# nv-tlabs/LION

Measured on NVIDIA H100. Metric: shapes/sec (1000-step DDPM, 2048 latent pts, B=32), higher is better.
Workload: dtype tf32 (fp32 storage/accumulate)

## Files before the change

### include/lion_b200.h

```cpp
#ifndef LION_B200_H
#define LION_B200_H
#include <stddef.h>
#ifdef __cplusplus
extern "C" {
#endif

typedef struct LionCtx LionCtx;
typedef struct LionModel LionModel;

int lion_version(void);
const char* lion_last_error(void);
int lion_ctx_create(int device, LionCtx** out);
int lion_ctx_destroy(LionCtx* ctx);
int lion_ctx_last_launches(LionCtx* ctx);
unsigned lion_ctx_generation(LionCtx* ctx);
int lion_ctx_timeline(LionCtx* ctx, unsigned long long* t_ns, char* names, int max_entries);
size_t lion_ctx_arena_bytes(LionCtx* ctx);
size_t lion_workspace_bytes(LionCtx* ctx);

int lion_avg_voxelize(const float* features, const int* coords, float* out, int* ind, int* cnt,
                      int B, int C, int N, int r, void* stream);
int lion_trilinear_devoxelize(const float* grid, const float* coords, float* out, int* inds, float* wgts,
                              int B, int C, int N, int r, int is_training, void* stream);
int lion_furthest_point_sampling(const float* coords, int* idx, int B, int N, int M, void* stream);
int lion_gather(const float* features, const int* idx, float* out, int B, int C, int N, int M, void* stream);
int lion_ball_query(const float* centers, const float* points, int* out, int B, int N, int M, float radius, int K,
                    void* stream);
int lion_grouping(const float* features, const int* idx, float* out, int B, int C, int N, int M, int U, void* stream);
int lion_three_nn_interpolate(const float* points, const float* centers, const float* centers_features, float* out,
                              int* idx, float* wgt, int B, int C, int N, int M, void* stream);
int lion_voxel_coords(const float* coords, float* norm_coords, int* vox, int B, int N, int r, int normalize, float eps,
                      void* stream);

int lion_avg_voxelize_backward(const float* grad_y , const int* ind , const int* cnt ,
                               float* grad_x , int B, int C, int N, int r, void* stream);
int lion_trilinear_devoxelize_backward(const float* grad_y , const int* inds , const float* wgts ,
                                       float* grad_x , int B, int C, int N, int r, void* stream);
int lion_grouping_backward(const float* grad_y , const int* idx , float* grad_x , int B, int C,
                           int N, int M, int U, void* stream);
int lion_three_nn_interpolate_backward(const float* grad_y , const int* idx , const float* wgt ,
                                       float* grad_x , int B, int C, int N, int M, void* stream);
int lion_gather_backward(const float* grad_y , const int* idx , float* grad_x , int B, int C, int N,
                         int M, void* stream);

enum { LION_KIND_UNET = 1, LION_KIND_PVCONV = 2, LION_KIND_SA = 3, LION_KIND_FP = 4, LION_KIND_ATTN = 5,
       LION_KIND_SHARED_MLP = 6, LION_KIND_GLOBAL_PRIOR = 7, LION_KIND_ADAGN = 8, LION_KIND_CONV3D = 9,
       LION_KIND_STYLE_ENC = 10 };
// ... 70 lines not shown
```

### lion_b200/_lib.py

```python
import ctypes as C
import os
import threading

import torch

_HERE = os.path.dirname(os.path.abspath(__file__))
LIB_PATH = os.path.join(_HERE, "csrc", "liblion_b200.so")


class LionError(RuntimeError):
    pass


_lib = None
_lock = threading.Lock()
c_f = C.c_void_p


def _proto(lib):
    i, f, sz, vp = C.c_int, C.c_float, C.c_size_t, C.c_void_p
    P = lambda *a: list(a)
    sig = {
        "lion_version": ([], i),
        "lion_last_error": ([], C.c_char_p),
        "lion_ctx_create": (P(i, C.POINTER(vp)), i),
        "lion_ctx_destroy": (P(vp), i),
        "lion_ctx_last_launches": (P(vp), i),
        "lion_ctx_arena_bytes": (P(vp), sz),
        "lion_ctx_generation": (P(vp), C.c_uint),
        "lion_ctx_timeline": (P(vp, vp, vp, i), i),
        "lion_avg_voxelize": (P(vp, vp, vp, vp, vp, i, i, i, i, vp), i),
        "lion_trilinear_devoxelize": (P(vp, vp, vp, vp, vp, i, i, i, i, i, vp), i),
        "lion_furthest_point_sampling": (P(vp, vp, i, i, i, vp), i),
        "lion_gather": (P(vp, vp, vp, i, i, i, i, vp), i),
        "lion_ball_query": (P(vp, vp, vp, i, i, i, f, i, vp), i),
        "lion_grouping": (P(vp, vp, vp, i, i, i, i, i, vp), i),
        "lion_three_nn_interpolate": (P(vp, vp, vp, vp, vp, vp, i, i, i, i, vp), i),
        "lion_voxel_coords": (P(vp, vp, vp, i, i, i, i, f, vp), i),
        "lion_avg_voxelize_backward": (P(vp, vp, vp, vp, i, i, i, i, vp), i),
        "lion_trilinear_devoxelize_backward": (P(vp, vp, vp, vp, i, i, i, i, vp), i),
        "lion_grouping_backward": (P(vp, vp, vp, i, i, i, i, i, vp), i),
        "lion_three_nn_interpolate_backward": (P(vp, vp, vp, vp, i, i, i, i, vp), i),
        "lion_gather_backward": (P(vp, vp, vp, i, i, i, i, vp), i),
        "lion_model_create": (P(vp, i, C.POINTER(i), i, C.POINTER(vp), i, C.POINTER(vp)), i),
        "lion_model_destroy": (P(vp), i),
        "lion_model_refresh": (P(vp), i),
        "lion_unet_forward": (P(vp, vp, vp, vp, vp, vp, i, i, vp), i),
        "lion_unet_cache_style": (P(vp, vp, vp, i, vp), i),
        "lion_style_encoder_forward": (P(vp, vp, vp, i, i, vp), i),
        "lion_pvconv_fwd": (P(vp, vp, vp, vp, vp, i, i, vp), i),
        "lion_sa_module_fwd": (P(vp, vp, vp, vp, vp, vp, i, i, vp), i),
        "lion_fp_module_fwd": (P(vp, vp, vp, vp, vp, vp, vp, i, i, i, vp), i),
        "lion_linear_attention_fwd": (P(vp, vp, vp, i, i, vp), i),
        "lion_shared_mlp_fwd": (P(vp, vp, vp, vp, i, i, vp), i),
        "lion_global_prior_forward": (P(vp, vp, vp, vp, vp, i, vp), i),
        "lion_adagn_fwd": (P(vp, vp, vp, vp, i, i, vp), i),
        "lion_se3d_fwd": (P(vp, vp, vp, vp, vp, i, i, i, vp), i),
        "lion_swish_fwd": (P(vp, vp, sz, vp), i),
        "lion_ddpm_update": (P(vp, vp, vp, vp, vp, vp, f, sz, vp, i, vp), i),
        "lion_ddpm_set_step": (P(vp, vp, i, i, vp), i),
# ... 178 lines not shown
```

### lion_b200/csrc/common.cuh

```cuda
#pragma once
#include <cuda_runtime.h>
#include <cstdint>
#include <cstdio>
#include <cstdarg>
#include <cstring>
#include <string>
#include <vector>
#include <mutex>

namespace lion {

enum : int { LION_OK = 0, LION_ERR_CUDA = -1, LION_ERR_ARG = -2, LION_ERR_OOM = -3, LION_ERR_STATE = -4 };

void set_error(const char* fmt, ...);
const char* get_error();

#define LION_CHECK_CUDA(expr)                                                          \
  do {                                                                                 \
    cudaError_t _e = (expr);                                                           \
    if (_e != cudaSuccess) {                                                           \
      lion::set_error("%s:%d: %s -> %s", __FILE__, __LINE__, #expr, cudaGetErrorString(_e)); \
      return lion::LION_ERR_CUDA;                                                      \
    }                                                                                  \
  } while (0)

#define LION_REQUIRE(cond, ...)                                                        \
  do {                                                                                 \
    if (!(cond)) {                                                                     \
      lion::set_error(__VA_ARGS__);                                                    \
      return lion::LION_ERR_ARG;                                                       \
    }                                                                                  \
  } while (0)

#define LION_TRY(expr)                                                                 \
  do {                                                                                 \
    int _r = (expr);                                                                   \
    if (_r != 0) return _r;                                                            \
  } while (0)

constexpr int LION_MAX_STAMPS = 256;
struct Ctx {
  int device = 0;
  int num_sms = 132;
  int l2_bytes = 50 << 20;
  cudaStream_t stream = nullptr;
  cudaStream_t aux = nullptr;
  char* base = nullptr;
  char* zgrid = nullptr;
  size_t zgrid_cap = 0, zgrid_need = 0;
  size_t cap = 0;
  size_t off = 0;
  size_t peak = 0;
  unsigned generation = 0;
  std::mutex* mu = nullptr;
  bool dry = false;
  int launches = 0;
  int conv_smem_cap = 0;
  unsigned long long* d_stamps = nullptr;
  int n_stamps = 0;
  char stamp_names[LION_MAX_STAMPS][24];

  void reset() { off = 0; peak = 0; launches = 0; zgrid_need = 0; n_stamps = 0; }
  void* alloc(size_t bytes) {
    size_t a = (off + 255) & ~size_t(255);
    off = a + bytes;
    if (off > peak) peak = off;
    if (dry) return (void*)(uintptr_t)(0x1000 + a);
    return base + a;
  }
  template <typename T> T* alloc_n(size_t n) { return (T*)alloc(n * sizeof(T)); }
  size_t mark() const { return off; }
  void release(size_t m) { off = m; }
};

int ctx_reserve(Ctx* c, size_t bytes);

#define LION_LAUNCH_ON(ctx, stream, kernel, grid, block, smem, ...)                    \
  do {                                                                                 \
    if (!(ctx)->dry) {                                                                 \
      kernel<<<(grid), (block), (smem), (stream)>>>(__VA_ARGS__);                      \
      (ctx)->launches++;                                                               \
    }                                                                                  \
  } while (0)
#define LION_LAUNCH(ctx, kernel, grid, block, smem, ...) LION_LAUNCH_ON(ctx, (ctx)->stream, kernel, grid, block, smem, __VA_ARGS__)

static __global__ void k_stamp(unsigned long long* p) {
  unsigned long long t;
  asm volatile("mov.u64 %0, %%globaltimer;" : "=l"(t));
  *p = t;
}
// ... 82 lines not shown
```

### lion_b200/csrc/conv_tc.cu

```cuda
#include <algorithm>

#include "common.cuh"
#include "model.cuh"
#include "wgmma.cuh"

namespace lion {
namespace tc {

using namespace sm90;

constexpr int CONSUMER_WARPS = 8;
constexpr int THREADS = 32 * CONSUMER_WARPS + 32;
constexpr int MAX_A_STAGES = 16;
constexpr int MAX_B_STAGES = 4;
constexpr int OCC_SMEM = 1024;
__host__ __device__ constexpr int tiles_per_item(int NT) { return NT <= 32 ? 4 : (NT <= 64 ? 2 : 1); }
constexpr int SMEM_BIAS = 128 * 4, SMEM_BARS = 64 * 8 + 128;
__host__ __device__ constexpr int smem_stat(int NT) { return CONSUMER_WARPS * 2 * NT * 4; }
__host__ __device__ constexpr int smem_pool(int NT, int TPG) { return TPG == 1 ? CONSUMER_WARPS * 2 * NT * 4 : 0; }
__host__ __device__ constexpr int smem_fixed(int NT, int TPG) {
  return SMEM_BIAS + smem_stat(NT) + smem_pool(NT, TPG) + SMEM_BARS + OCC_SMEM;
}

struct Params {
  const float4* in; const float* w; const float* bias; float4* out; double* ssum; double* ssq;
  int Gin, Gout_store, cout_pad;
  int rows;
  int p_begin, p_end;
  int ntile;
  int ntg, tpg;
  int tg_off[3];
  int tap_off[9];
  int r, rp, nzb, npl, nblk, ib;
  int halo;
  int KG, nchunk;
  int NT;
  int G;
  int B;
  int a_stage_bytes, b_stage_bytes, stage_rows;
  int a_stages;
  int b_stages;
  const unsigned char* occ;
  int occ_stride;
  float* pool_mm;
  int sched;
};

__host__ __device__ __forceinline__ int block_row(int k, int rp, int nzb, int npl) {
  const int x = k / npl, rem = k - x * npl, yb = rem / nzb, zb = rem - yb * nzb;
  return ((x + 1) * rp + 1 + 8 * yb) * rp + 1 + 8 * zb;
}

template <int KG, int TPG, int NT>
__device__ __forceinline__ void issue_stage(float* d, uint32_t a_addr, uint32_t b_addr, uint32_t a_pitch, uint32_t a_sbo,
                                            const int* tap_off) {
  const uint64_t a0 = make_desc(a_addr, a_pitch, a_sbo), b0 = make_desc(b_addr, NT * 16, 128);
#pragma unroll
  for (int t = 0; t < TPG; ++t) {
    const uint64_t at = a0 + (uint64_t)(int64_t)(TPG == 1 ? 0 : tap_off[t]);
#pragma unroll
    for (int ks = 0; ks < KG / 2; ++ks)
      wgmma_tf32<NT>(d, at + (uint64_t)((ks * 2 * a_pitch) >> 4), b0 + (uint64_t)(((t * KG + ks * 2) * NT * 16) >> 4), 1);
  }
}


struct Items {
  long long u, u_end; int ntile_total, B, G;
  int mode, m, q, n_p, n_q, c_i, i, big, k;
  __device__ __forceinline__ bool next(int& nt, long long& v0, int& ntile) {
    const long long per_nt = (long long)B * ntile_total;
    if (mode) {
      while (u >= u_end) {
        if (k >= m) return false;
        const int a0 = q * k / m, a1 = q * (k + 1) / m, b0 = (q + 1) * k / m, b1 = (q + 1) * (k + 1) / m;
        u = (long long)n_q * a0 + (long long)n_p * b0 + (long long)(i - c_i) * (a1 - a0) + (long long)c_i * (b1 - b0);
        u_end = u + (big ? b1 - b0 : a1 - a0);
        ++k;
      }
      nt = (int)(u / per_nt);
      v0 = u - (long long)nt * per_nt;
      const long long lim = (long long)(nt + 1) * per_nt;
      const long long e = u_end < lim ? u_end : lim;
      ntile = (int)(e - u);
      u = e;
      return true;
    }
    if (u >= u_end) return false;
    nt = (int)(u / per_nt);
    v0 = u - (long long)nt * per_nt;
    long long run = per_nt - v0;
    if (u_end - u < run) run = u_end - u;
    const long long k2 = (run + G - 1) / G;
    ntile = (int)((run + k2 - 1) / k2);
    u += ntile;
// ... 15 lines not shown
}

__device__ __forceinline__ void halo_mask(int p_lo, int rp, bool& ok_lo, bool& ok_hi) {
  const int p_hi = p_lo + 8;
  const int z0 = p_lo % rp, y0 = (p_lo / rp) % rp, z1 = p_hi % rp, y1 = (p_hi / rp) % rp;
  ok_lo = ok_lo && z0 >= 1 && z0 <= rp - 2 && y0 >= 1 && y0 <= rp - 2;
  ok_hi = ok_hi && z1 >= 1 && z1 <= rp - 2 && y1 >= 1 && y1 <= rp - 2;
}
template <int NT>
__device__ __forceinline__ void stat_add(float* s_stat, int cw, int lane, int col, float x0, float x1, float x2, float x3) {
  const float s0 = red8<0>(x0 + x2), s1 = red8<0>(x1 + x3);
  const float q0 = red8<0>(fmaf(x0, x0, x2 * x2)), q1 = red8<0>(fmaf(x1, x1, x3 * x3));
  if (lane < 4) {
    float* st = s_stat + (cw * 2) * NT + col;
    st[0] += s0; st[1] += s1; st[NT] += q0; st[NT + 1] += q1;
  }
}
template <int NT>
__device__ __forceinline__ void stat_flush(const Params& P, float* s_stat, int et, int b, int n0) {
  asm volatile("bar.sync 1, 256;" ::: "memory");
  if (et < NT) {
    float s = 0.f, qq = 0.f;
#pragma unroll
    for (int w = 0; w < CONSUMER_WARPS; ++w) {
      s += s_stat[(w * 2 + 0) * NT + et]; qq += s_stat[(w * 2 + 1) * NT + et];
      s_stat[(w * 2 + 0) * NT + et] = 0.0f; s_stat[(w * 2 + 1) * NT + et] = 0.0f;
    }
    atomicAdd(P.ssum + (size_t)b * P.cout_pad + n0 + et, (double)s);
    atomicAdd(P.ssq + (size_t)b * P.cout_pad + n0 + et, (double)qq);
  }
  asm volatile("bar.sync 1, 256;" ::: "memory");
}

template <int KG, int TPG, int NT, bool BLK>
__global__ void __launch_bounds__(THREADS, 1) k_conv_tc(Params P) {
  constexpr int GT = tiles_per_item(NT);
  constexpr int NACC = NT / 2;
  extern __shared__ __align__(128) uint8_t smem[];
  uint8_t* sA = smem;
  const int A_STAGES = P.a_stages;
  uint8_t* sB = sA + (size_t)A_STAGES * P.a_stage_bytes;
  const int B_STAGES = P.b_stages;
  float* s_bias = (float*)(sB + (size_t)B_STAGES * P.b_stage_bytes);
  float* s_stat = s_bias + 128;
  float* s_pool = s_stat + CONSUMER_WARPS * 2 * NT;
  uint64_t* bars = (uint64_t*)((uint8_t*)s_stat + smem_stat(NT) + smem_pool(NT, TPG));
  volatile uint32_t* s_skip = (volatile uint32_t*)(bars + 64);
  uint8_t* s_occ = (uint8_t*)(bars + 64) + 128;
  const int tid = threadIdx.x, warp = tid >> 5, lane = tid & 31;

  const uint32_t bar_full_a = smem_u32(bars), bar_empty_a = smem_u32(bars + MAX_A_STAGES);
  const uint32_t bar_full_b = smem_u32(bars + 2 * MAX_A_STAGES), bar_empty_b = smem_u32(bars + 2 * MAX_A_STAGES + MAX_B_STAGES);

  if (P.Gin % KG != 0)
    for (int i = tid; i < A_STAGES * P.a_stage_bytes / 16; i += THREADS) ((float4*)sA)[i] = make_float4(0.f, 0.f, 0.f, 0.f);
  for (int i = tid; i < CONSUMER_WARPS * 2 * NT; i += THREADS) s_stat[i] = 0.0f;
  if (tid == 0) {
    for (int i = 0; i < A_STAGES; ++i) { mbar_init(bar_full_a + 8 * i, 1); mbar_init(bar_empty_a + 8 * i, CONSUMER_WARPS); }
    for (int i = 0; i < B_STAGES; ++i) { mbar_init(bar_full_b + 8 * i, 1); mbar_init(bar_empty_b + 8 * i, CONSUMER_WARPS); }
    asm volatile("fence.mbarrier_init.release.cluster;" ::: "memory");
  }
  asm volatile("fence.proxy.async.shared::cta;" ::: "memory");
  __syncthreads();

  const int ntile_total = P.ntile;
  const int n_nt = P.cout_pad / P.NT;
  const long long U = (long long)n_nt * P.B * ntile_total;
  const Items items0 = make_items(U, ntile_total, P.B, P.G, P.sched);

  if (warp == CONSUMER_WARPS) {
    uint32_t sa = 0, pa = 0, sb = 0, pb = 0;
    const uint32_t bytes = (uint32_t)P.stage_rows * 16u;
    const uint32_t sA_addr = smem_u32(sA), sB_addr = smem_u32(sB);
    Items items = items0;
    int nt, ntile;
    long long v0;
    int occ_shape = -1;
    while (items.next(nt, v0, ntile)) {
      const float* wsrc = P.w + (size_t)nt * P.nchunk * P.ntg * (P.b_stage_bytes / 4);
      int my_b = 0, my_t = 0;
      if (lane < ntile) { const int vl = (int)v0 + lane; my_b = vl / ntile_total; my_t = vl - my_b * ntile_total; }
      for (int cc = 0; cc < P.nchunk; ++cc) {
        const int kg_real = min(KG, P.Gin - cc * KG);
        const size_t grp_lane = (size_t)(cc * KG + (lane < kg_real ? lane : 0));
        for (int tg = 0; tg < P.ntg; ++tg) {
          const bool may_skip = P.occ && !(cc == P.nchunk - 1 && tg == P.ntg - 1);
          mbar_wait(bar_empty_b + 8 * sb, pb ^ 1);
          if (lane == 0) {
            mbar_expect_tx(bar_full_b + 8 * sb, P.b_stage_bytes);
            bulk_g2s(sB_addr + sb * (uint32_t)P.b_stage_bytes, wsrc + (size_t)(cc * P.ntg + tg) * (P.b_stage_bytes / 4),
                     P.b_stage_bytes, bar_full_b + 8 * sb);
          }
          if (++sb == B_STAGES) { sb = 0; pb ^= 1; }
          for (int j = 0; j < ntile; ++j) {
            const int bj = __shfl_sync(0xffffffffu, my_b, j), tj = __shfl_sync(0xffffffffu, my_t, j);
            long long row0;
            uint32_t cnt = (uint32_t)P.stage_rows;
            if (!BLK) {
              row0 = (long long)P.p_begin + (long long)tj * 128 - P.halo + P.tg_off[tg];
            } else {
              row0 = (long long)block_row(tj * P.ib, P.rp, P.nzb, P.npl) - P.rp - 1 + P.tg_off[tg];
              if (row0 + cnt > (long long)P.rows) cnt = (uint32_t)(P.rows - row0);
            }
            const float4* in_lane = P.in + ((size_t)bj * P.Gin + grp_lane) * P.rows;
            mbar_wait(bar_empty_a + 8 * sa, pa ^ 1);
            bool empty = false;
            if (may_skip) {
              const unsigned char* occ_b = P.occ + (size_t)bj * P.occ_stride;
              if (P.occ_stride <= OCC_SMEM) {
                if (occ_shape != bj) {
                  __syncwarp();
                  for (int k = lane; k < P.occ_stride; k += 32) s_occ[k] = __ldg(occ_b + k);
                  __syncwarp();
                  occ_shape = bj;
                }
                occ_b = s_occ;
              }
              long long lo = row0 < 0 ? 0 : row0, hi = row0 + cnt - 1;
              if (hi > P.rows - 1) hi = P.rows - 1;
              unsigned any = 0;
              for (int k = (int)(lo >> 6); k <= (int)(hi >> 6); ++k) any |= occ_b[k];
              empty = (any == 0);
            }
            const uint32_t full = bar_full_a + 8 * sa;
            if (lane == 0) {
              s_skip[sa] = empty ? 1u : 0u;
              if (empty) asm volatile("mbarrier.arrive.release.cta.shared::cta.b64 _, [%0];" ::"r"(full) : "memory");
              else mbar_expect_tx(full, cnt * 16u * kg_real);
            }
            __syncwarp();
            if (!empty && lane < kg_real)
              bulk_g2s(sA_addr + sa * (uint32_t)P.a_stage_bytes + lane * bytes, in_lane + row0, cnt * 16u, full);
            if (++sa == (uint32_t)A_STAGES) { sa = 0; pa ^= 1; }
          }
        }
      }
    }
  } else {
    const int cw = warp, wg = cw >> 2, wq = cw & 3;
    const int et = tid;
    const uint32_t a_pitch = (uint32_t)P.stage_rows * 16u;
    const uint32_t a_sbo = BLK ? (uint32_t)P.rp * 16u : 128u;
    const uint32_t a_ring = smem_u32(sA) + (BLK ? 0u : (uint32_t)(P.halo + 64 * wg) * 16u);
    const uint32_t b_ring = smem_u32(sB);
    const int r_lo = 64 * wg + 16 * wq + (lane >> 2);
    const int c_lo = 2 * (lane & 3);
    const bool odd = (lane & 1) != 0;
    float acc[GT][NACC];
    uint32_t sa = 0, pa = 0, sb = 0, pb = 0;
    Items items = items0;
    int nt, ntile;
    long long v0;
    auto release = [&](int& s, uint32_t bar0) {
      if (s >= 0) { if (lane == 0) mbar_arrive(bar0 + 8 * s); s = -1; }
    };
    while (items.next(nt, v0, ntile)) {
#pragma unroll
      for (int j = 0; j < GT; ++j)
#pragma unroll
        for (int i = 0; i < NACC; ++i) acc[j][i] = 0.0f;
      int g_f = 0, nbw = 0;
      uint32_t boff[GT];
      if (BLK) {
        const int g_b = (int)(v0 / ntile_total);
        g_f = (int)(v0 - (long long)g_b * ntile_total) * P.ib;
        const int nb = min(P.ib, P.nblk - g_f);
        nbw = (nb - wg + 1) / 2;
        const int s_f = block_row(g_f, P.rp, P.nzb, P.npl);
#pragma unroll
        for (int j = 0; j < GT; ++j) {
          const int k = 2 * j + wg < nb ? g_f + 2 * j + wg : g_f;
          boff[j] = (uint32_t)(block_row(k, P.rp, P.nzb, P.npl) - s_f + P.rp + 1) * 16u;
        }
      }
      int pend_a = -1, pend_b = -1;
      for (int cc = 0; cc < P.nchunk; ++cc) {
        for (int tg = 0; tg < P.ntg; ++tg) {
          mbar_wait(bar_full_b + 8 * sb, pb);
          const uint32_t b_addr = b_ring + sb * (uint32_t)P.b_stage_bytes;
#pragma unroll
          for (int j = 0; j < (BLK ? 1 : GT); ++j) {
            if (j < ntile) {
              mbar_wait(bar_full_a + 8 * sa, pa);
              const uint32_t a_addr = a_ring + sa * (uint32_t)P.a_stage_bytes;
              if (!s_skip[sa]) {
                wg_fence();
                if (!BLK) {
                  issue_stage<KG, TPG, NT>(acc[j], a_addr, b_addr, a_pitch, a_sbo, P.tap_off);
                } else {
#pragma unroll
                  for (int k = 0; k < GT; ++k) issue_stage<KG, TPG, NT>(acc[k], a_addr + boff[k], b_addr, a_pitch, a_sbo, P.tap_off);
                }
                wg_commit();
                wg_wait<1>();
                release(pend_a, bar_empty_a);
                release(pend_b, bar_empty_b);
                pend_a = (int)sa;
              } else {
                int s = (int)sa;
                release(s, bar_empty_a);
              }
              if (++sa == (uint32_t)A_STAGES) { sa = 0; pa ^= 1; }
            }
          }
          if (pend_b >= 0) {
            wg_wait<0>();
            release(pend_a, bar_empty_a);
            release(pend_b, bar_empty_b);
          }
          if (pend_a >= 0) pend_b = (int)sb;
          else { int s = (int)sb; release(s, bar_empty_b); }
          if (++sb == B_STAGES) { sb = 0; pb ^= 1; }
        }
      }
      wg_wait<0>();
      release(pend_a, bar_empty_a);
      release(pend_b, bar_empty_b);
#pragma unroll
      for (int j = 0; j < GT; ++j) fence_regs<NACC>(acc[j]);

      const int n0 = nt * NT;
      asm volatile("bar.sync 1, 256;" ::: "memory");
      if (et < NT) s_bias[et] = P.bias ? P.bias[n0 + et] : 0.0f;
      asm volatile("bar.sync 1, 256;" ::: "memory");
// ... 161 lines not shown
  if (!w.tc.w) return false;
  if (geo.ntaps != w.ntaps) return false;
  return true;
}

int conv_tc_run(Ctx* c, const ConvW& w, const float4* in, int Gin, float4* out, int Gout_store, double* ssum, double* ssq,
                const ConvGeom& geo, int B, float* pool_mm) {
  tc::Params P{};
  if (pool_mm && (w.ntaps != 1 || geo.p_begin != 0 || geo.p_end != geo.rows || geo.rows % 128)) {
    set_error("conv_tc: the pooled epilogue needs a 1x1 convolution over a multiple of 128 rows"); return LION_ERR_ARG;
  }
  P.pool_mm = pool_mm;
  const int NT = w.tc.NT, KG = w.tc.KG, tpg = w.tc.tpg;
  P.in = in; P.w = w.tc.w; P.bias = w.bias; P.out = out; P.ssum = ssum; P.ssq = ssq;
  P.Gin = Gin; P.Gout_store = Gout_store; P.cout_pad = w.cout_pad;
  P.rows = geo.rows; P.p_begin = geo.p_begin; P.p_end = geo.p_end;
  P.ntg = w.tc.ntg; P.tpg = tpg; P.KG = KG; P.nchunk = w.tc.nchunk; P.NT = NT;
  P.b_stage_bytes = tpg * KG * NT * 16;
  P.B = B;
  P.occ = geo.occ; P.occ_stride = geo.occ_stride;
  const size_t fixed = tc::smem_fixed(NT, tpg);
  const bool blk = w.ntaps == 27 && NT == 128;
  const int ntile_rows = cdiv(geo.p_end - geo.p_begin, 128);
  int ntile;
  P.halo = 0;
  if (w.ntaps == 27) {
    const int rp = geo.rp, r = rp - 2;
    for (int dx = 0; dx < 3; ++dx) P.tg_off[dx] = (dx - 1) * rp * rp;
    for (int dy = 0; dy < 3; ++dy) for (int dz = 0; dz < 3; ++dz) P.tap_off[dy * 3 + dz] = (dy - 1) * rp + (dz - 1);
    P.r = r; P.rp = rp;
  } else {
    P.tg_off[0] = 0; P.tap_off[0] = 0;
  }
  if (blk) {
    const int rp = P.rp, r = P.r;
    P.nzb = cdiv(r, 8); P.npl = P.nzb * P.nzb; P.nblk = r * P.npl;
    const int ib = 2 * tc::tiles_per_item(NT);
    int wrows = 0;
    for (int f = 0; f < P.nblk; f += ib) {
      const int l = std::min(f + ib, P.nblk) - 1;
      wrows = std::max(wrows, tc::block_row(l, rp, P.nzb, P.npl) - tc::block_row(f, rp, P.nzb, P.npl) + 9 * rp + 10);
    }
    P.ib = ib;
    P.stage_rows = wrows;
    ntile = cdiv(P.nblk, ib);
    P.G = 1;
  } else {
    if (w.ntaps == 27) P.halo = P.rp + 1;
    P.stage_rows = 128 + 2 * P.halo;
    ntile = ntile_rows;
    P.G = tc::tiles_per_item(NT);
  }
  P.ntile = ntile;
  P.a_stage_bytes = KG * P.stage_rows * 16;
  int b_stages = 2;
  if (blk) {
    const long long limit = (c->conv_smem_cap > 0 ? c->conv_smem_cap : 227LL * 1024) - (long long)fixed;
    while (b_stages < tc::MAX_B_STAGES &&
           (limit - (long long)(b_stages + 1) * P.b_stage_bytes) / P.a_stage_bytes >= std::max(4, b_stages + 1))
      ++b_stages;
  }
  P.b_stages = b_stages;
  const long long a_room = 227LL * 1024 - (long long)fixed - (long long)b_stages * P.b_stage_bytes;
  int n_tiles_n = w.cout_pad / NT;
  const double in_bytes = (double)B * Gin * geo.rows * 16.0;
  P.sched = w.ntaps == 27 && in_bytes > 1.6 * c->l2_bytes ? 1 : 0;
  int a_stages = (int)(a_room / P.a_stage_bytes);
  if (c->conv_smem_cap > 0 && a_stages >= 5) {
    int capped = (int)(((long long)c->conv_smem_cap - (long long)fixed - (long long)b_stages * P.b_stage_bytes) / P.a_stage_bytes);
    if (capped >= 4 && capped < a_stages) a_stages = capped;
  }
  if (a_stages > tc::MAX_A_STAGES) a_stages = tc::MAX_A_STAGES;
  if (a_stages < 2) { set_error("conv_tc: shared memory cannot hold the operand pipeline (N=%d, KG=%d)", NT, KG); return LION_ERR_ARG; }
  P.a_stages = a_stages;
  size_t smem = (size_t)a_stages * P.a_stage_bytes + (size_t)b_stages * P.b_stage_bytes + fixed;
  if (smem > 227 * 1024) { set_error("conv_tc: %zu bytes of shared memory needed", smem); return LION_ERR_ARG; }
  auto grid_for = [&](int nt_per_shape) {
    long long n_units = (long long)nt_per_shape * n_tiles_n * B;
    long long per_cta = (n_units + c->num_sms - 1) / c->num_sms;
    return (int)((n_units + per_cta - 1) / per_cta);
  };
  const int grid = grid_for(ntile);
  tc::Params S = P;
  if (blk && ssum) {
    P.ssum = nullptr; P.ssq = nullptr;
    S.ntile = ntile_rows; S.G = tc::tiles_per_item(NT);
  }
  auto stats = [&]() -> int {
    if (!(blk && ssum)) return 0;
    LION_LAUNCH(c, tc::k_conv_stats<128>, grid_for(ntile_rows), 256, 0, S);
    return check_launch(c, "conv_tc stats");
  };
#define CONV_TC_CASE(kg, tpg_, nt_, blk_)                                                                 \
  if (KG == kg && tpg == tpg_ && NT == nt_ && blk == blk_) {                                              \
    static DevOnce attr_once;                                                                             \
    if (attr_once.need()) {                                                                               \
      LION_CHECK_CUDA(cudaFuncSetAttribute(tc::k_conv_tc<kg, tpg_, nt_, blk_>, cudaFuncAttributeMaxDynamicSharedMemorySize, 227 * 1024)); \
    }                                                                                                     \
    LION_LAUNCH(c, (tc::k_conv_tc<kg, tpg_, nt_, blk_>), grid, tc::THREADS, smem, P);                     \
    LION_TRY(check_launch(c, "conv_tc"));                                                                 \
    return stats();                                                                                       \
  }
#define CONV_TC_NT(kg, tpg_) CONV_TC_CASE(kg, tpg_, 32, false) CONV_TC_CASE(kg, tpg_, 64, false) CONV_TC_CASE(kg, tpg_, 96, false)
  CONV_TC_NT(2, 1) CONV_TC_NT(4, 1) CONV_TC_NT(8, 1) CONV_TC_NT(2, 9) CONV_TC_NT(4, 9) CONV_TC_NT(8, 9)
  CONV_TC_CASE(2, 1, 128, false) CONV_TC_CASE(4, 1, 128, false) CONV_TC_CASE(8, 1, 128, false)
  CONV_TC_CASE(2, 9, 128, true) CONV_TC_CASE(4, 9, 128, true)
#undef CONV_TC_NT
#undef CONV_TC_CASE
  set_error("conv_tc: no kernel for N=%d, KG=%d, %d taps", NT, KG, tpg);
  return LION_ERR_ARG;
}

}
```

### lion_b200/csrc/net.cu

```cuda
#include <algorithm>
#include <deque>
#include <memory>
#include <cstdlib>
#include <cmath>
#include "common.cuh"
#include "packed_kernels.cuh"
#include "model.cuh"
#include "../../include/lion_b200.h"

namespace lion {

static thread_local char g_err[1024] = "";
void set_error(const char* fmt, ...) {
  va_list ap;
  va_start(ap, fmt);
  vsnprintf(g_err, sizeof(g_err), fmt, ap);
  va_end(ap);
}
const char* get_error() { return g_err; }

int ctx_reserve(Ctx* c, size_t bytes) {
  if (bytes <= c->cap) return 0;
  cudaStreamCaptureStatus st = cudaStreamCaptureStatusNone;
  cudaStreamIsCapturing(c->stream, &st);
// ... 944 lines not shown
extern "C" const char* lion_last_error(void) { return get_error(); }

extern "C" int lion_ctx_create(int device, LionCtx** out) {
  LION_REQUIRE(out, "lion_ctx_create: null out");
  LION_CHECK_CUDA(cudaSetDevice(device));
  LionCtx* h = new LionCtx();
  h->c.device = device;
  h->c.mu = &h->mu;
  cudaDeviceProp prop;
  LION_CHECK_CUDA(cudaGetDeviceProperties(&prop, device));
  h->c.num_sms = prop.multiProcessorCount;
  h->c.l2_bytes = prop.l2CacheSize;
  LION_CHECK_CUDA(cudaStreamCreateWithFlags(&h->c.aux, cudaStreamNonBlocking));
  { const char* e = getenv("LION_TIMELINE");
    if (e && atoi(e) != 0) LION_CHECK_CUDA(cudaMalloc(&h->c.d_stamps, LION_MAX_STAMPS * sizeof(unsigned long long))); }
  if (prop.major != 9 || prop.minor != 0) {
    set_error("lion_b200 is built for sm_90a only; device %d is sm_%d%d", device, prop.major, prop.minor);
    delete h;
    return LION_ERR_STATE;
  }
  *out = h;
  return 0;
}
extern "C" int lion_ctx_destroy(LionCtx* h) {
  if (!h) return 0;
  if (h->c.base) cudaFree(h->c.base);
  if (h->c.zgrid) cudaFree(h->c.zgrid);
  if (h->c.aux) cudaStreamDestroy(h->c.aux);
  if (h->c.d_stamps) cudaFree(h->c.d_stamps);
  delete h;
  return 0;
}
extern "C" int lion_ctx_last_launches(LionCtx* h) { return h ? h->c.launches : 0; }
extern "C" unsigned lion_ctx_generation(LionCtx* h) { return h ? h->c.generation : 0; }
extern "C" int lion_ctx_timeline(LionCtx* h, unsigned long long* t_ns, char* names, int max_entries) {
  LION_REQUIRE(h && t_ns && names && max_entries >= 0, "lion_ctx_timeline: null argument");
  if (!h->c.d_stamps) { set_error("lion_ctx_timeline: the context was created without LION_TIMELINE=1"); return LION_ERR_STATE; }
  int n = h->c.n_stamps < max_entries ? h->c.n_stamps : max_entries;
  LION_CHECK_CUDA(cudaSetDevice(h->c.device));
  LION_CHECK_CUDA(cudaDeviceSynchronize());
  LION_CHECK_CUDA(cudaMemcpy(t_ns, h->c.d_stamps, (size_t)n * sizeof(unsigned long long), cudaMemcpyDeviceToHost));
  for (int i = 0; i < n; ++i) memcpy(names + (size_t)i * 24, h->c.stamp_names[i], 24);
  return n;
}
extern "C" size_t lion_ctx_arena_bytes(LionCtx* h) { return h ? h->c.cap : 0; }
extern "C" size_t lion_workspace_bytes(LionCtx* h) { return h ? h->c.cap + h->c.zgrid_cap : 0; }

extern "C" int lion_model_create(LionCtx* ctx, int kind, const int* desc, int ndesc, const float* const* params,
                                 int nparams, LionModel** out) {
  LION_REQUIRE(ctx && out && (desc || ndesc == 0) && (params || nparams == 0), "lion_model_create: null argument");
  LION_CHECK_CUDA(cudaSetDevice(ctx->c.device));
  std::unique_ptr<LionModel> h(new LionModel());
  Model* m = &h->m;
  m->ctx = &ctx->c; m->kind = kind;
  m->desc.assign(desc, desc + ndesc);
  m->params.assign(params, params + nparams);
  for (int i = 0; i < nparams; ++i) LION_REQUIRE(params[i], "lion_model_create: parameter %d is null", i);
  Cursor cur{m->params.data(), nparams};
  const std::vector<int>& d = m->desc;
  auto need = [&](int n) { return (int)d.size() >= n; };
  switch (kind) {
    case LION_KIND_UNET: LION_TRY(build_unet(m, cur)); break;
    case LION_KIND_PVCONV: {
      LION_REQUIRE(need(5), "pvconv descriptor: [cin, cout, r, attn, style_dim]");
      m->S = d[4] > 0 ? d[4] : 4;
      m->block.reset(new Block()); m->block->kind = kind;
// ... 346 lines not shown
```

### lion_b200/csrc/wgmma.cuh

```cuda
#pragma once
#include <cstdint>

namespace lion {
namespace sm90 {

__device__ __forceinline__ uint32_t smem_u32(const void* p) { return (uint32_t)__cvta_generic_to_shared(p); }
__device__ __forceinline__ void mbar_init(uint32_t bar, uint32_t count) {
  asm volatile("mbarrier.init.shared::cta.b64 [%0], %1;" ::"r"(bar), "r"(count));
}
__device__ __forceinline__ void mbar_expect_tx(uint32_t bar, uint32_t bytes) {
  asm volatile("mbarrier.arrive.expect_tx.shared::cta.b64 _, [%0], %1;" ::"r"(bar), "r"(bytes) : "memory");
}
__device__ __forceinline__ void mbar_arrive(uint32_t bar) {
  asm volatile("mbarrier.arrive.release.cta.shared::cta.b64 _, [%0];" ::"r"(bar) : "memory");
}
__device__ __forceinline__ bool mbar_try(uint32_t bar, uint32_t parity) {
  uint32_t ok;
  asm volatile("{\n.reg .pred p;\nmbarrier.try_wait.parity.shared::cta.b64 p, [%1], %2;\nselp.u32 %0, 1, 0, p;\n}"
               : "=r"(ok) : "r"(bar), "r"(parity) : "memory");
  return ok != 0;
}
static __device__ __noinline__ void mbar_wait_slow(uint32_t bar, uint32_t parity) {
  long long t0 = clock64();
  while (!mbar_try(bar, parity)) {
    if (clock64() - t0 > 2000000000LL) __trap();
  }
}
__device__ __forceinline__ void mbar_wait(uint32_t bar, uint32_t parity) {
  if (!mbar_try(bar, parity)) mbar_wait_slow(bar, parity);
  __syncwarp();
}
__device__ __forceinline__ void bulk_g2s(uint32_t dst, const void* src, uint32_t bytes, uint32_t bar) {
  asm volatile("cp.async.bulk.shared::cluster.global.mbarrier::complete_tx::bytes [%0], [%1], %2, [%3];"
               ::"r"(dst), "l"(src), "r"(bytes), "r"(bar) : "memory");
}

__device__ __forceinline__ uint64_t make_desc(uint32_t addr, uint32_t lbo_bytes, uint32_t sbo_bytes) {
  uint64_t d = 0;
  d |= (uint64_t)((addr >> 4) & 0x3fff);
  d |= (uint64_t)((lbo_bytes >> 4) & 0x3fff) << 16;
  d |= (uint64_t)((sbo_bytes >> 4) & 0x3fff) << 32;
  return d;
}

__device__ __forceinline__ void wg_fence() { asm volatile("wgmma.fence.sync.aligned;" ::: "memory"); }
__device__ __forceinline__ void wg_commit() { asm volatile("wgmma.commit_group.sync.aligned;" ::: "memory"); }
template <int N>
__device__ __forceinline__ void wg_wait() { asm volatile("wgmma.wait_group.sync.aligned %0;" ::"n"(N) : "memory"); }
template <int R>
__device__ __forceinline__ void fence_regs(float* d) {
#pragma unroll
  for (int i = 0; i < R; ++i) asm volatile("" : "+f"(d[i])::"memory");
}

template <int OP>
__device__ __forceinline__ float red8(float v) {
#pragma unroll
  for (int o = 4; o < 32; o <<= 1) {
    const float g = __shfl_xor_sync(0xffffffffu, v, o);
    v = OP == 0 ? v + g : (OP == 1 ? fminf(v, g) : fmaxf(v, g));
  }
  return v;
}

template <int N> __device__ __forceinline__ void wgmma_tf32(float* d, uint64_t a, uint64_t b, int scale_d);
template <> __device__ __forceinline__ void wgmma_tf32<32>(float* d, uint64_t a, uint64_t b, int scale_d) {
  asm volatile("{\n.reg .pred p;\nsetp.ne.b32 p, %18, 0;\n"
               "wgmma.mma_async.sync.aligned.m64n32k8.f32.tf32.tf32 {%0, %1, %2, %3, %4, %5, %6, %7, %8, %9, %10, %11, %12, %13, %14, %15}, %16, %17, p, 1, 1;\n}\n"
               : "+f"(d[0]), "+f"(d[1]), "+f"(d[2]), "+f"(d[3]), "+f"(d[4]), "+f"(d[5]), "+f"(d[6]), "+f"(d[7]), "+f"(d[8]), "+f"(d[9]), "+f"(d[10]), "+f"(d[11]), "+f"(d[12]), "+f"(d[13]), "+f"(d[14]), "+f"(d[15])
               : "l"(a), "l"(b), "r"(scale_d));
}
template <> __device__ __forceinline__ void wgmma_tf32<64>(float* d, uint64_t a, uint64_t b, int scale_d) {
  asm volatile("{\n.reg .pred p;\nsetp.ne.b32 p, %34, 0;\n"
               "wgmma.mma_async.sync.aligned.m64n64k8.f32.tf32.tf32 {%0, %1, %2, %3, %4, %5, %6, %7, %8, %9, %10, %11, %12, %13, %14, %15, %16, %17, %18, %19, %20, %21, %22, %23, %24, %25, %26, %27, %28, %29, %30, %31}, %32, %33, p, 1, 1;\n}\n"
               : "+f"(d[0]), "+f"(d[1]), "+f"(d[2]), "+f"(d[3]), "+f"(d[4]), "+f"(d[5]), "+f"(d[6]), "+f"(d[7]), "+f"(d[8]), "+f"(d[9]), "+f"(d[10]), "+f"(d[11]), "+f"(d[12]), "+f"(d[13]), "+f"(d[14]), "+f"(d[15]), "+f"(d[16]), "+f"(d[17]), "+f"(d[18]), "+f"(d[19]), "+f"(d[20]), "+f"(d[21]), "+f"(d[22]), "+f"(d[23]), "+f"(d[24]), "+f"(d[25]), "+f"(d[26]), "+f"(d[27]), "+f"(d[28]), "+f"(d[29]), "+f"(d[30]), "+f"(d[31])
               : "l"(a), "l"(b), "r"(scale_d));
// ... 17 lines not shown
```

Baseline: 2.835.

## Group four spatial blocks per conv tile with warp-specialized register reallocation

For the blocked 27-tap 3D conv path, each CTA can now process four 8x8 spatial blocks per A-stage instead of two, chosen when the grid still fills the SMs and at least three A stages fit in shared memory. Each B (weight) stage is then reused across more output tiles. To hold the larger accumulator set, the kernel adds a full producer warpgroup and uses setmaxnreg to move registers from producer to consumers. Waits are inlined in that variant. Risks are fewer pipeline stages from the larger windows, register pressure, and fewer CTAs. A debug accessor reports the chosen group size.

```diff
diff --git a/include/lion_b200.h b/include/lion_b200.h
--- a/include/lion_b200.h
+++ b/include/lion_b200.h
@@ -13,6 +13,7 @@
 int lion_ctx_create(int device, LionCtx** out);
 int lion_ctx_destroy(LionCtx* ctx);
 int lion_ctx_last_launches(LionCtx* ctx);
+int lion_ctx_last_conv_group(LionCtx* ctx);
 unsigned lion_ctx_generation(LionCtx* ctx);
 int lion_ctx_timeline(LionCtx* ctx, unsigned long long* t_ns, char* names, int max_entries);
 size_t lion_ctx_arena_bytes(LionCtx* ctx);
diff --git a/lion_b200/_lib.py b/lion_b200/_lib.py
--- a/lion_b200/_lib.py
+++ b/lion_b200/_lib.py
@@ -26,6 +26,7 @@
         "lion_ctx_create": (P(i, C.POINTER(vp)), i),
         "lion_ctx_destroy": (P(vp), i),
         "lion_ctx_last_launches": (P(vp), i),
+        "lion_ctx_last_conv_group": (P(vp), i),
         "lion_ctx_arena_bytes": (P(vp), sz),
         "lion_ctx_generation": (P(vp), C.c_uint),
         "lion_ctx_timeline": (P(vp, vp, vp, i), i),
diff --git a/lion_b200/csrc/common.cuh b/lion_b200/csrc/common.cuh
--- a/lion_b200/csrc/common.cuh
+++ b/lion_b200/csrc/common.cuh
@@ -56,6 +56,7 @@
   bool dry = false;
   int launches = 0;
   int conv_smem_cap = 0;
+  int conv_group_blocks = 0;
   unsigned long long* d_stamps = nullptr;
   int n_stamps = 0;
   char stamp_names[LION_MAX_STAMPS][24];
diff --git a/lion_b200/csrc/conv_tc.cu b/lion_b200/csrc/conv_tc.cu
--- a/lion_b200/csrc/conv_tc.cu
+++ b/lion_b200/csrc/conv_tc.cu
@@ -11,6 +11,8 @@
 
 constexpr int CONSUMER_WARPS = 8;
 constexpr int THREADS = 32 * CONSUMER_WARPS + 32;
+__host__ __device__ constexpr int conv_threads(int BPW) { return BPW == 2 ? 32 * CONSUMER_WARPS + 128 : THREADS; }
+constexpr int PRODUCER_REGS = 96, CONSUMER_REGS = 200;
 constexpr int MAX_A_STAGES = 16;
 constexpr int MAX_B_STAGES = 4;
 constexpr int OCC_SMEM = 1024;
@@ -51,16 +53,21 @@
   return ((x + 1) * rp + 1 + 8 * yb) * rp + 1 + 8 * zb;
 }
 
-template <int KG, int TPG, int NT>
-__device__ __forceinline__ void issue_stage(float* d, uint32_t a_addr, uint32_t b_addr, uint32_t a_pitch, uint32_t a_sbo,
-                                            const int* tap_off) {
-  const uint64_t a0 = make_desc(a_addr, a_pitch, a_sbo), b0 = make_desc(b_addr, NT * 16, 128);
+template <int KG, int TPG, int NT, int NB = 1>
+__device__ __forceinline__ void issue_stage(float (*d)[NT / 2], const uint32_t* a_addr, uint32_t b_addr, uint32_t a_pitch,
+                                            uint32_t a_sbo, const int* tap_off) {
+  const uint64_t b0 = make_desc(b_addr, NT * 16, 128);
+  uint64_t a0[NB];
+#pragma unroll
+  for (int k = 0; k < NB; ++k) a0[k] = make_desc(a_addr[k], a_pitch, a_sbo);
 #pragma unroll
   for (int t = 0; t < TPG; ++t) {
-    const uint64_t at = a0 + (uint64_t)(int64_t)(TPG == 1 ? 0 : tap_off[t]);
+    const uint64_t toff = (uint64_t)(int64_t)(TPG == 1 ? 0 : tap_off[t]);
 #pragma unroll
     for (int ks = 0; ks < KG / 2; ++ks)
-      wgmma_tf32<NT>(d, at + (uint64_t)((ks * 2 * a_pitch) >> 4), b0 + (uint64_t)(((t * KG + ks * 2) * NT * 16) >> 4), 1);
+#pragma unroll
+      for (int k = 0; k < NB; ++k)
+        wgmma_tf32<NT>(d[k], a0[k] + toff + (uint64_t)((ks * 2 * a_pitch) >> 4), b0 + (uint64_t)(((t * KG + ks * 2) * NT * 16) >> 4), 1);
   }
 }
 
@@ -142,9 +149,11 @@
   asm volatile("bar.sync 1, 256;" ::: "memory");
 }
 
-template <int KG, int TPG, int NT, bool BLK>
-__global__ void __launch_bounds__(THREADS, 1) k_conv_tc(Params P) {
-  constexpr int GT = tiles_per_item(NT);
+template <int KG, int TPG, int NT, bool BLK, int BPW = 1>
+__global__ void __launch_bounds__(conv_threads(BPW), 1) k_conv_tc(Params P) {
+  constexpr int GT = BLK ? BPW : tiles_per_item(NT);
+  constexpr int NTHR = conv_threads(BPW);
+  constexpr bool SETREG = NTHR > THREADS;
   constexpr int NACC = NT / 2;
   extern __shared__ __align__(128) uint8_t smem[];
   uint8_t* sA = smem;
@@ -163,8 +172,8 @@
   const uint32_t bar_full_b = smem_u32(bars + 2 * MAX_A_STAGES), bar_empty_b = smem_u32(bars + 2 * MAX_A_STAGES + MAX_B_STAGES);
 
   if (P.Gin % KG != 0)
-    for (int i = tid; i < A_STAGES * P.a_stage_bytes / 16; i += THREADS) ((float4*)sA)[i] = make_float4(0.f, 0.f, 0.f, 0.f);
-  for (int i = tid; i < CONSUMER_WARPS * 2 * NT; i += THREADS) s_stat[i] = 0.0f;
+    for (int i = tid; i < A_STAGES * P.a_stage_bytes / 16; i += NTHR) ((float4*)sA)[i] = make_float4(0.f, 0.f, 0.f, 0.f);
+  for (int i = tid; i < CONSUMER_WARPS * 2 * NT; i += NTHR) s_stat[i] = 0.0f;
   if (tid == 0) {
     for (int i = 0; i < A_STAGES; ++i) { mbar_init(bar_full_a + 8 * i, 1); mbar_init(bar_empty_a + 8 * i, CONSUMER_WARPS); }
     for (int i = 0; i < B_STAGES; ++i) { mbar_init(bar_full_b + 8 * i, 1); mbar_init(bar_empty_b + 8 * i, CONSUMER_WARPS); }
@@ -178,7 +187,11 @@
   const long long U = (long long)n_nt * P.B * ntile_total;
   const Items items0 = make_items(U, ntile_total, P.B, P.G, P.sched);
 
-  if (warp == CONSUMER_WARPS) {
+  if (warp >= CONSUMER_WARPS) {
+    if constexpr (SETREG) {
+      regs_dec<PRODUCER_REGS>();
+      if (warp > CONSUMER_WARPS) return;
+    }
     uint32_t sa = 0, pa = 0, sb = 0, pb = 0;
     const uint32_t bytes = (uint32_t)P.stage_rows * 16u;
     const uint32_t sA_addr = smem_u32(sA), sB_addr = smem_u32(sB);
@@ -195,7 +208,7 @@
         const size_t grp_lane = (size_t)(cc * KG + (lane < kg_real ? lane : 0));
         for (int tg = 0; tg < P.ntg; ++tg) {
           const bool may_skip = P.occ && !(cc == P.nchunk - 1 && tg == P.ntg - 1);
-          mbar_wait(bar_empty_b + 8 * sb, pb ^ 1);
+          mbar_wait<SETREG>(bar_empty_b + 8 * sb, pb ^ 1);
           if (lane == 0) {
             mbar_expect_tx(bar_full_b + 8 * sb, P.b_stage_bytes);
             bulk_g2s(sB_addr + sb * (uint32_t)P.b_stage_bytes, wsrc + (size_t)(cc * P.ntg + tg) * (P.b_stage_bytes / 4),
@@ -213,7 +226,7 @@
               if (row0 + cnt > (long long)P.rows) cnt = (uint32_t)(P.rows - row0);
             }
             const float4* in_lane = P.in + ((size_t)bj * P.Gin + grp_lane) * P.rows;
-            mbar_wait(bar_empty_a + 8 * sa, pa ^ 1);
+            mbar_wait<SETREG>(bar_empty_a + 8 * sa, pa ^ 1);
             bool empty = false;
             if (may_skip) {
               const unsigned char* occ_b = P.occ + (size_t)bj * P.occ_stride;
@@ -247,6 +260,7 @@
       }
     }
   } else {
+    if constexpr (SETREG) regs_inc<CONSUMER_REGS>();
     const int cw = warp, wg = cw >> 2, wq = cw & 3;
     const int et = tid;
     const uint32_t a_pitch = (uint32_t)P.stage_rows * 16u;
@@ -286,20 +300,22 @@
       int pend_a = -1, pend_b = -1;
       for (int cc = 0; cc < P.nchunk; ++cc) {
         for (int tg = 0; tg < P.ntg; ++tg) {
-          mbar_wait(bar_full_b + 8 * sb, pb);
+          mbar_wait<SETREG>(bar_full_b + 8 * sb, pb);
           const uint32_t b_addr = b_ring + sb * (uint32_t)P.b_stage_bytes;
 #pragma unroll
           for (int j = 0; j < (BLK ? 1 : GT); ++j) {
             if (j < ntile) {
-              mbar_wait(bar_full_a + 8 * sa, pa);
+              mbar_wait<SETREG>(bar_full_a + 8 * sa, pa);
               const uint32_t a_addr = a_ring + sa * (uint32_t)P.a_stage_bytes;
               if (!s_skip[sa]) {
                 wg_fence();
                 if (!BLK) {
-                  issue_stage<KG, TPG, NT>(acc[j], a_addr, b_addr, a_pitch, a_sbo, P.tap_off);
+                  issue_stage<KG, TPG, NT>(&acc[j], &a_addr, b_addr, a_pitch, a_sbo, P.tap_off);
                 } else {
-#pragma unroll
-                  for (int k = 0; k < GT; ++k) issue_stage<KG, TPG, NT>(acc[k], a_addr + boff[k], b_addr, a_pitch, a_sbo, P.tap_off);
+                  uint32_t a_blk[GT];
+#pragma unroll
+                  for (int k = 0; k < GT; ++k) a_blk[k] = a_addr + boff[k];
+                  issue_stage<KG, TPG, NT, GT>(acc, a_blk, b_addr, a_pitch, a_sbo, P.tap_off);
                 }
                 wg_commit();
                 wg_wait<1>();
@@ -527,18 +543,23 @@
   } else {
     P.tg_off[0] = 0; P.tap_off[0] = 0;
   }
+  const int n_tiles_n = w.cout_pad / NT;
   if (blk) {
     const int rp = P.rp, r = P.r;
     P.nzb = cdiv(r, 8); P.npl = P.nzb * P.nzb; P.nblk = r * P.npl;
-    const int ib = 2 * tc::tiles_per_item(NT);
-    int wrows = 0;
-    for (int f = 0; f < P.nblk; f += ib) {
-      const int l = std::min(f + ib, P.nblk) - 1;
-      wrows = std::max(wrows, tc::block_row(l, rp, P.nzb, P.npl) - tc::block_row(f, rp, P.nzb, P.npl) + 9 * rp + 10);
-    }
-    P.ib = ib;
-    P.stage_rows = wrows;
-    ntile = cdiv(P.nblk, ib);
+    auto window_rows = [&](int ib) {
+      int wrows = 0;
+      for (int f = 0; f < P.nblk; f += ib) {
+        const int l = std::min(f + ib, P.nblk) - 1;
+        wrows = std::max(wrows, tc::block_row(l, rp, P.nzb, P.npl) - tc::block_row(f, rp, P.nzb, P.npl) + 9 * rp + 10);
+      }
+      return wrows;
+    };
+    const long long a_room2 = 227LL * 1024 - (long long)fixed - 2LL * P.b_stage_bytes;
+    const bool four = (long long)n_tiles_n * B * cdiv(P.nblk, 4) >= c->num_sms && a_room2 / (KG * window_rows(4) * 16) >= 3;
+    P.ib = four ? 4 : 2;
+    P.stage_rows = window_rows(P.ib);
+    ntile = cdiv(P.nblk, P.ib);
     P.G = 1;
   } else {
     if (w.ntaps == 27) P.halo = P.rp + 1;
@@ -557,7 +578,6 @@
   }
   P.b_stages = b_stages;
   const long long a_room = 227LL * 1024 - (long long)fixed - (long long)b_stages * P.b_stage_bytes;
-  int n_tiles_n = w.cout_pad / NT;
   const double in_bytes = (double)B * Gin * geo.rows * 16.0;
   P.sched = w.ntaps == 27 && in_bytes > 1.6 * c->l2_bytes ? 1 : 0;
   int a_stages = (int)(a_room / P.a_stage_bytes);
@@ -586,20 +606,22 @@
     LION_LAUNCH(c, tc::k_conv_stats<128>, grid_for(ntile_rows), 256, 0, S);
     return check_launch(c, "conv_tc stats");
   };
-#define CONV_TC_CASE(kg, tpg_, nt_, blk_)                                                                 \
-  if (KG == kg && tpg == tpg_ && NT == nt_ && blk == blk_) {                                              \
+  const int bpw = blk ? P.ib / 2 : 1;
+  c->conv_group_blocks = blk ? P.ib : 0;
+#define CONV_TC_CASE(kg, tpg_, nt_, blk_, bpw_)                                                           \
+  if (KG == kg && tpg == tpg_ && NT == nt_ && blk == blk_ && bpw == bpw_) {                               \
     static DevOnce attr_once;                                                                             \
     if (attr_once.need()) {                                                                               \
-      LION_CHECK_CUDA(cudaFuncSetAttribute(tc::k_conv_tc<kg, tpg_, nt_, blk_>, cudaFuncAttributeMaxDynamicSharedMemorySize, 227 * 1024)); \
+      LION_CHECK_CUDA(cudaFuncSetAttribute(tc::k_conv_tc<kg, tpg_, nt_, blk_, bpw_>, cudaFuncAttributeMaxDynamicSharedMemorySize, 227 * 1024)); \
     }                                                                                                     \
-    LION_LAUNCH(c, (tc::k_conv_tc<kg, tpg_, nt_, blk_>), grid, tc::THREADS, smem, P);                     \
+    LION_LAUNCH(c, (tc::k_conv_tc<kg, tpg_, nt_, blk_, bpw_>), grid, tc::conv_threads(bpw_), smem, P);    \
     LION_TRY(check_launch(c, "conv_tc"));                                                                 \
     return stats();                                                                                       \
   }
-#define CONV_TC_NT(kg, tpg_) CONV_TC_CASE(kg, tpg_, 32, false) CONV_TC_CASE(kg, tpg_, 64, false) CONV_TC_CASE(kg, tpg_, 96, false)
+#define CONV_TC_NT(kg, tpg_) CONV_TC_CASE(kg, tpg_, 32, false, 1) CONV_TC_CASE(kg, tpg_, 64, false, 1) CONV_TC_CASE(kg, tpg_, 96, false, 1)
   CONV_TC_NT(2, 1) CONV_TC_NT(4, 1) CONV_TC_NT(8, 1) CONV_TC_NT(2, 9) CONV_TC_NT(4, 9) CONV_TC_NT(8, 9)
-  CONV_TC_CASE(2, 1, 128, false) CONV_TC_CASE(4, 1, 128, false) CONV_TC_CASE(8, 1, 128, false)
-  CONV_TC_CASE(2, 9, 128, true) CONV_TC_CASE(4, 9, 128, true)
+  CONV_TC_CASE(2, 1, 128, false, 1) CONV_TC_CASE(4, 1, 128, false, 1) CONV_TC_CASE(8, 1, 128, false, 1)
+  CONV_TC_CASE(2, 9, 128, true, 1) CONV_TC_CASE(4, 9, 128, true, 1) CONV_TC_CASE(2, 9, 128, true, 2) CONV_TC_CASE(4, 9, 128, true, 2)
 #undef CONV_TC_NT
 #undef CONV_TC_CASE
   set_error("conv_tc: no kernel for N=%d, KG=%d, %d taps", NT, KG, tpg);
diff --git a/lion_b200/csrc/net.cu b/lion_b200/csrc/net.cu
--- a/lion_b200/csrc/net.cu
+++ b/lion_b200/csrc/net.cu
@@ -1000,6 +1000,7 @@
   return 0;
 }
 extern "C" int lion_ctx_last_launches(LionCtx* h) { return h ? h->c.launches : 0; }
+extern "C" int lion_ctx_last_conv_group(LionCtx* h) { return h ? h->c.conv_group_blocks : 0; }
 extern "C" unsigned lion_ctx_generation(LionCtx* h) { return h ? h->c.generation : 0; }
 extern "C" int lion_ctx_timeline(LionCtx* h, unsigned long long* t_ns, char* names, int max_entries) {
   LION_REQUIRE(h && t_ns && names && max_entries >= 0, "lion_ctx_timeline: null argument");
diff --git a/lion_b200/csrc/wgmma.cuh b/lion_b200/csrc/wgmma.cuh
--- a/lion_b200/csrc/wgmma.cuh
+++ b/lion_b200/csrc/wgmma.cuh
@@ -26,8 +26,18 @@
     if (clock64() - t0 > 2000000000LL) __trap();
   }
 }
+template <bool INLINE = false>
 __device__ __forceinline__ void mbar_wait(uint32_t bar, uint32_t parity) {
-  if (!mbar_try(bar, parity)) mbar_wait_slow(bar, parity);
+  if (!mbar_try(bar, parity)) {
+    if constexpr (INLINE) {
+      const long long t0 = clock64();
+      while (!mbar_try(bar, parity)) {
+        if (clock64() - t0 > 2000000000LL) __trap();
+      }
+    } else {
+      mbar_wait_slow(bar, parity);
+    }
+  }
   __syncwarp();
 }
 __device__ __forceinline__ void bulk_g2s(uint32_t dst, const void* src, uint32_t bytes, uint32_t bar) {
@@ -42,6 +52,11 @@
   d |= (uint64_t)((sbo_bytes >> 4) & 0x3fff) << 32;
   return d;
 }
+
+template <int R>
+__device__ __forceinline__ void regs_dec() { asm volatile("setmaxnreg.dec.sync.aligned.u32 %0;" ::"n"(R)); }
+template <int R>
+__device__ __forceinline__ void regs_inc() { asm volatile("setmaxnreg.inc.sync.aligned.u32 %0;" ::"n"(R)); }
 
 __device__ __forceinline__ void wg_fence() { asm volatile("wgmma.fence.sync.aligned;" ::: "memory"); }
 __device__ __forceinline__ void wg_commit() { asm volatile("wgmma.commit_group.sync.aligned;" ::: "memory"); }
```

Result: faster. 2.929 (median of 6 runs) (+3.3%).
